# YichengDWu/tinyedm

Hardware: AMD Instinct MI355X
Metric: train imgs/sec CIFAR-10 32x32 bf16 (higher is better)
Workload: dtype bf16; 1 GPU; CIFAR-10 32x32 unconditional EDM2 U-Net (conf/cifar10.yaml, 35.6M params) full training step: diffuse+embed+denoiser fwd/bwd+loss+grad all-reduce+Adam+EMA; per_gpu_batch=128, global_batch=128, parallelism=dp1, conditional=False, step_launch=hipGraph replay, collective=none

## Files before the change

include/tinyedm_hip.h:

```cpp
#ifndef TINYEDM_HIP_H
#define TINYEDM_HIP_H
#ifdef __cplusplus
extern "C" {
#endif

typedef struct ihipStream_t* edm_stream_t;

int edm_version(void);
const char* edm_last_error(void);
int edm_init(int device);
int edm_graph_replay_safe(void);
typedef struct {
  unsigned step, seed_lo, seed_hi, reserved;
  float lr, ema_beta, grad_scale, bc1, bc2sqrt, pad[3];
} edm_step_params;

int edm_conv_igemm(const void* X, const void* Wp, void* Y, const void* R, float alpha, float beta, int B, int H,
                   int W, int Cin, int Cout, int taps, edm_stream_t stream);
int edm_conv_igemm_v2(const void* X, const void* Wp, void* Y, const void* R, float alpha, float beta, int B, int H,
                      int W, int Cin, int Cout, int taps, edm_stream_t stream);
int edm_conv_igemm_v6(const void* X, const void* Wp, void* Y, const void* R, float alpha, float beta, int B, int H,
                      int W, int Cin, int Cout, int taps, edm_stream_t stream);
int edm_conv_igemm_s(const void* X, const void* Wp, void* Y, const void* R, float alpha, float beta, int B, int H,
                     int W, int Cin, int Cout, int taps, edm_stream_t stream);
// ... 68 lines not shown
} edm_finish_item;
long edm_wgrad_finish_multi_table_bytes(void);
int edm_wgrad_finish_multi(const edm_finish_item* items, int n, void* table_host, void* table_dev, int defer_upload,
                           edm_stream_t stream);

int edm_attention_fwd(const void* qkv, void* y, int B, int N, int C, int heads, edm_stream_t stream);
int edm_attention_bwd(const void* qkv, const void* y, const void* gy, void* gqkv, int B, int N, int C, int heads,
                      edm_stream_t stream);

int edm_attention_qkv_supported(int N, int C, int heads);
int edm_attention_qkv_fwd(const void* x, const void* Wqkv, void* y, void* stat, int B, int N, int C, int heads,
                          int heads_per_wg, edm_stream_t stream);
int edm_attention_qkv_bwd(const void* x, const void* y, const void* gout, const void* stat, const void* Wqkv,
                          const void* Wd_out, void* gqkv, float alpha, int B, int N, int C, int heads, int heads_per_wg,
                          edm_stream_t stream);

int edm_pixelnorm_silu_fwd(const void* x, void* xn, void* a, float* dsave, long P, int C, edm_stream_t stream);
int edm_pixelnorm_silu_bwd(const void* xn, const float* dsave, const void* gxn, float gxn_scale, const void* ga,
                           const void* gadd, void* gx, long P, int C, edm_stream_t stream);
int edm_pool_pixelnorm_silu_fwd(const void* x, void* xn, void* a, float* dsave, int B, int Hp, int Wp, int C,
                                edm_stream_t stream);
int edm_pool_pixelnorm_silu_bwd(const void* xn, const float* dsave, const void* gxn, float gxn_scale, const void* ga,
                                const void* gadd, void* gx, int B, int Hp, int Wp, int C, edm_stream_t stream);
int edm_silu_fwd(const void* x, void* a, long n, edm_stream_t stream);
int edm_silu_bwd(const void* x, const void* ga, const void* gextra, float extra_scale, void* gx, long n,
                 edm_stream_t stream);
int edm_axpby(const void* a, float alpha, const void* b, float beta, void* out, long n, edm_stream_t stream);
int edm_mod_silu_drop_fwd(const void* r, const float* lin, long lin_stride, const float* gain, void* a, int B, int HW,
                          int C, float pdrop, unsigned long long seed, unsigned sub, unsigned step, const void* dyn,
                          edm_stream_t stream);
int edm_mod_silu_drop_bwd(const void* r, const float* lin, long lin_stride, const float* gain, const void* ga, void* gr,
                          float* gm, float* glin, long glin_stride, float* ggain, int B, int HW, int C, float pdrop,
                          unsigned long long seed, unsigned sub, unsigned step, const void* dyn, edm_stream_t stream);
int edm_mod_silu_drop_bwd_raw(const void* r, const float* lin, long lin_stride, const float* gain, const void* ga, void* gr,
                              float* gm, long gm_stride, int B, int HW, int C, float pdrop, unsigned long long seed,
                              unsigned sub, unsigned step, const void* dyn, edm_stream_t stream);
int edm_dropout_mask(unsigned char* mask, long n, float pdrop, unsigned long long seed, unsigned sub, unsigned step,
                     edm_stream_t stream);
int edm_pool2(const void* x, void* y, int B, int Hout, int Wout, int C, float scale, edm_stream_t stream);
int edm_up2(const void* x, const void* add, void* y, int B, int Hout, int Wout, int C, float scale, edm_stream_t stream);
int edm_up2_silu(const void* x, void* y, void* a, int B, int Hout, int Wout, int C, edm_stream_t stream);
int edm_reduce_hw(const void* x, long x_stride, const void* y, long y_stride, float* out, int B, int HW, int C,
                  float scale, edm_stream_t stream);
int edm_scalelong_fwd(const float* mean, const float* W1h, const float* W2h, float* gate, float* z1save, int B, int C,
                      int R, edm_stream_t stream);
int edm_scalelong_bwd(const float* mean, const float* W1h, const float* W2h, const float* gate, const float* z1save,
// ... 200 lines not shown
```

tinyedm_amd/_lib.py:

```python
import ctypes
import os

_HERE = os.path.dirname(os.path.abspath(__file__))
LIB_PATH = os.environ.get("EDM_LIB_PATH") or os.path.join(_HERE, "libtinyedm_hip.so")

P, I, L, F = ctypes.c_void_p, ctypes.c_int, ctypes.c_long, ctypes.c_float
U, U64 = ctypes.c_uint, ctypes.c_ulonglong

SIGNATURES = {
    "edm_version": [],
    "edm_last_error": [],
    "edm_init": [I],
    "edm_graph_replay_safe": [],
    "edm_pixelnorm_silu_fwd": [P, P, P, P, L, I, P],
    "edm_pixelnorm_silu_bwd": [P, P, P, F, P, P, P, L, I, P],
    "edm_pool_pixelnorm_silu_fwd": [P, P, P, P, I, I, I, I, P],
    "edm_pool_pixelnorm_silu_bwd": [P, P, P, F, P, P, P, I, I, I, I, P],
    "edm_up2_silu": [P, P, P, I, I, I, I, P],
    "edm_silu_fwd": [P, P, L, P],
    "edm_silu_bwd": [P, P, P, F, P, L, P],
    "edm_axpby": [P, F, P, F, P, L, P],
    "edm_mod_silu_drop_fwd": [P, P, L, P, P, I, I, I, F, U64, U, U, P, P],
    "edm_mod_silu_drop_bwd": [P, P, L, P, P, P, P, P, L, P, I, I, I, F, U64, U, U, P, P],
    "edm_mod_silu_drop_bwd_raw": [P, P, L, P, P, P, P, L, I, I, I, F, U64, U, U, P, P],
    "edm_dropout_mask": [P, L, F, U64, U, U, P],
    "edm_pool2": [P, P, I, I, I, I, F, P],
    "edm_up2": [P, P, P, I, I, I, I, F, P],
    "edm_reduce_hw": [P, L, P, L, P, I, I, I, F, P],
    "edm_scalelong_fwd": [P, P, P, P, P, I, I, I, P],
    "edm_scalelong_bwd": [P, P, P, P, P, P, P, P, P, I, I, I, P],
    "edm_skip_gate_fwd": [P, P, P, P, P, P, I, I, I, I, P],
    "edm_skip_gate_bwd": [P, L, I, P, P, P, P, P, P, P, P, P, P, I, I, I, I, P],
    "edm_skip_gate_wgrad_multi": [P, I, P, P, I, P],
    "edm_skip_gate_wgrad_multi_table_bytes": [],
    "edm_skip_gate_fwd_multi": [P, I, P, P, I, P],
    "edm_skip_gate_fwd_multi_table_bytes": [],
    "edm_skip_gate_bwd_multi": [P, I, P, P, I, P],
    "edm_skip_half_bwd_multi": [P, I, P, P, I, P],
    "edm_skip_gate_bwd_multi_table_bytes": [],
    "edm_concat_gate_fwd": [P, P, P, P, P, I, I, I, I, P],
# ... 193 lines not shown
```

tinyedm_amd/csrc/elementwise.hip:

```cpp
#include "common.h"
#include <stdarg.h>
#include <stdio.h>

static thread_local char g_err[512] = "";
extern "C" void edm_set_error(const char* fmt, ...) {
  va_list ap;
  va_start(ap, fmt);
  vsnprintf(g_err, sizeof(g_err), fmt, ap);
  va_end(ap);
}
extern "C" const char* edm_last_error() { return g_err; }
extern "C" int edm_version() { return 1; }

static inline int cdiv(long a, long b) { return (int)((a + b - 1) / b); }
static inline int grid_for(long work, int block, int cap = 256 * 16) {
  long g = (work + block - 1) / block;
  if (g > cap) g = cap;
  if (g < 1) g = 1;
  return (int)g;
}

template <int LPP, bool POOL = false>
__global__ __launch_bounds__(256) void k_pnorm_silu_fwd(const bf16* __restrict__ x, bf16* __restrict__ xn,
                                                          bf16* __restrict__ a, float* __restrict__ dsave, int P,
// ... 35 lines not shown
      }
    }
    ss = group_sum<LPP>(ss);
    const float d = NORM_EPS + sqrtf(ss) * rsC;
    const float inv = 1.0f / d;
#pragma unroll
    for (int it = 0; it < 2; ++it) {
      const int c8 = lig + it * LPP;
      if (pv && c8 < CL) {
        float o[8], s[8];
#pragma unroll
        for (int i = 0; i < 8; ++i) {
          o[i] = (float)(bf16)(v[it][i] * inv);
          s[i] = mp_silu_b(o[i]);
        }
        store8(xn + p * C + c8 * 8, o);
        store8(a + p * C + c8 * 8, s);
      }
    }
    if (pv && lig == 0) dsave[p] = d;
  }
}

template <int LPP, bool UP = false>
__global__ __launch_bounds__(256) void k_pnorm_silu_bwd(const bf16* __restrict__ xn, const float* __restrict__ dsave,
                                                          const bf16* __restrict__ gxn, float gs,
                                                          const bf16* __restrict__ ga, const bf16* __restrict__ gadd,
                                                          bf16* __restrict__ gx, int P, int C, int Hp = 0, int Wp = 0) {
  constexpr int GPW = 64 / LPP;
  const int lane = threadIdx.x & 63, wave = threadIdx.x >> 6;
  const int lig = lane % LPP, grp = lane / LPP;
  const int CL = C >> 3;
  const long stride = (long)gridDim.x * 4 * GPW;
  for (long p0 = ((long)blockIdx.x * 4 + wave) * GPW; p0 < P; p0 += stride) {
    const long p = p0 + grp;
    const bool pv = p < P;
    float y[2][8], g[2][8];
    float dot = 0.f;
#pragma unroll
    for (int it = 0; it < 2; ++it) {
      const int c8 = lig + it * LPP;
      if (pv && c8 < CL) {
        load8(xn + p * C + c8 * 8, y[it]);
        float t[8];
        if (gxn) {
          load8(gxn + p * C + c8 * 8, t);
#pragma unroll
          for (int i = 0; i < 8; ++i) g[it][i] = gs * t[i];
        } else {
#pragma unroll
          for (int i = 0; i < 8; ++i) g[it][i] = 0.f;
// ... 8 lines not shown
      }
    }
    dot = group_sum<LPP>(dot);
    float d = pv ? dsave[p] : 1.f;
    float s = d - NORM_EPS;
    float coef = s > 0.f ? dot * d / ((float)C * s) : 0.f;
    float inv = 1.0f / d;
#pragma unroll
    for (int it = 0; it < 2; ++it) {
      const int c8 = lig + it * LPP;
      if (pv && c8 < CL) {
        float o[8];
#pragma unroll
        for (int i = 0; i < 8; ++i) o[i] = (g[it][i] - y[it][i] * coef) * inv;
        if constexpr (UP) {
          const int w = (int)(p % Wp);
          const long t2 = p / Wp;
          const int h = (int)(t2 % Hp);
          const long b = t2 / Hp;
          const long e0 = ((b * 2 * Hp + 2 * h) * 2 * Wp + 2 * w) * C + c8 * 8;
          const long row = (long)2 * Wp * C;
#pragma unroll
          for (int i = 0; i < 8; ++i) o[i] = 0.25f * (float)(bf16)o[i];
#pragma unroll
          for (int q = 0; q < 4; ++q) {
            const long e = e0 + (q >> 1) * row + (q & 1) * C;
            float r[8];
#pragma unroll
            for (int i = 0; i < 8; ++i) r[i] = o[i];
            if (gadd) {
              float t[8];
              load8(gadd + e, t);
#pragma unroll
              for (int i = 0; i < 8; ++i) r[i] += t[i];
            }
            store8(gx + e, r);
          }
          continue;
        }
        if (gadd) {
          float t[8];
          load8(gadd + p * C + c8 * 8, t);
#pragma unroll
          for (int i = 0; i < 8; ++i) o[i] += t[i];
        }
        store8(gx + p * C + c8 * 8, o);
      }
    }
  }
}

static int pick_lpp(int C) {
  int cl = C / 8;
  return cl <= 16 ? 16 : (cl <= 32 ? 32 : 64);
}

extern "C" int edm_pixelnorm_silu_fwd(const void* x, void* xn, void* a, float* dsave, long P, int C,
                                      hipStream_t st) {
  EDM_REQUIRE(P > 0 && P < (1L << 31) && C > 0 && C % 8 == 0 && C <= 1024, "pixelnorm_silu_fwd: bad P=%ld C=%d", P, C);
  int lpp = pick_lpp(C);
  int gpw = 64 / lpp;
  int grid = grid_for(P, 4 * gpw);
#define L(N) hipLaunchKernelGGL(k_pnorm_silu_fwd<N>, dim3(grid), dim3(256), 0, st, (const bf16*)x, (bf16*)xn, (bf16*)a, dsave, (int)P, C)
// ... 23 lines not shown
  EDM_REQUIRE(xn && dsave && gx && B > 0 && Hp > 0 && Wp > 0 && C > 0 && C % 8 == 0 && C <= 1024 &&
                  (long)B * Hp * Wp < (1L << 31), "pool_pixelnorm_silu_bwd: bad args");
  const long P = (long)B * Hp * Wp;
  int lpp = pick_lpp(C);
  int gpw = 64 / lpp;
  int grid = grid_for(P, 4 * gpw);
#define L(N) hipLaunchKernelGGL((k_pnorm_silu_bwd<N, true>), dim3(grid), dim3(256), 0, st, (const bf16*)xn, dsave, (const bf16*)gxn, gxn_scale, (const bf16*)ga, (const bf16*)gadd, (bf16*)gx, (int)P, C, Hp, Wp)
  if (lpp == 16) L(16); else if (lpp == 32) L(32); else L(64);
#undef L
  EDM_CHECK_LAUNCH("pool_pixelnorm_silu_bwd");
  return EDM_OK;
}

extern "C" int edm_pixelnorm_silu_bwd(const void* xn, const float* dsave, const void* gxn, float gxn_scale,
                                      const void* ga, const void* gadd, void* gx, long P, int C, hipStream_t st) {
  EDM_REQUIRE(P > 0 && P < (1L << 31) && C > 0 && C % 8 == 0 && C <= 1024, "pixelnorm_silu_bwd: bad P=%ld C=%d", P, C);
  int lpp = pick_lpp(C);
  int gpw = 64 / lpp;
  int grid = grid_for(P, 4 * gpw);
#define L(N) hipLaunchKernelGGL(k_pnorm_silu_bwd<N>, dim3(grid), dim3(256), 0, st, (const bf16*)xn, dsave, (const bf16*)gxn, gxn_scale, (const bf16*)ga, (const bf16*)gadd, (bf16*)gx, (int)P, C)
  if (lpp == 16) L(16); else if (lpp == 32) L(32); else L(64);
#undef L
  EDM_CHECK_LAUNCH("pixelnorm_silu_bwd");
  return EDM_OK;
}

__global__ void k_silu_fwd(const bf16* __restrict__ x, bf16* __restrict__ a, long n8) {
  for (long i = (long)blockIdx.x * blockDim.x + threadIdx.x; i < n8; i += (long)gridDim.x * blockDim.x) {
    float v[8];
    load8(x + i * 8, v);
#pragma unroll
    for (int j = 0; j < 8; ++j) v[j] = mp_silu_b(v[j]);
    store8(a + i * 8, v);
  }
}
__global__ void k_silu_bwd(const bf16* __restrict__ x, const bf16* __restrict__ ga, const bf16* __restrict__ ge,
                           float s, bf16* __restrict__ gx, long n8) {
  for (long i = (long)blockIdx.x * blockDim.x + threadIdx.x; i < n8; i += (long)gridDim.x * blockDim.x) {
    float v[8], g[8], e[8];
    load8(x + i * 8, v);
    load8(ga + i * 8, g);
    if (ge) load8(ge + i * 8, e);
#pragma unroll
    for (int j = 0; j < 8; ++j) g[j] = mp_silu_grad_b(v[j]) * g[j] + (ge ? s * e[j] : 0.f);
    store8(gx + i * 8, g);
  }
// ... 649 lines not shown
  int k = 0;
  const int n = g->n;
  while (k + 1 < n && (int)blockIdx.x >= g->it[k + 1].blk0) ++k;
  const SgbItem it = g->it[k];
  const int C = g->C, b = (int)blockIdx.x - it.blk0;
  skip_gate_bwd_body(it.gcat, it.gs, it.skip, it.W1, it.W2, it.gate, it.z1, it.gmean, it.ws, it.HW, C, it.R, b);
  if (it.gskip == nullptr) return;
  __syncthreads();
  const int CLs = C >> 3;
  const float inv_hw = 1.0f / (float)it.HW;
  const bf16* __restrict__ gc = it.gcat + (long)b * it.HW * it.gs;
  bf16* __restrict__ out = it.gskip + (long)b * it.HW * C;
  const float* gp0 = it.gate + (long)b * C;
  const float* mp0 = it.gmean + (long)b * C;
  const int n8 = it.HW * CLs;
  for (int i = threadIdx.x; i < n8; i += blockDim.x) {
    const int cs = (i % CLs) * 8;
    const int pix = i / CLs;
    float v[8];
    load8(gc + (long)pix * it.gs + cs, v);
    const float* gp = gp0 + cs;
    const float* mp = mp0 + cs;
#pragma unroll
    for (int j = 0; j < 8; ++j) v[j] = v[j] * gp[j] + mp[j] * inv_hw;
    store8(out + (long)pix * C + cs, v);
  }
}
__device__ __forceinline__ void skip_gate_wgrad_body(const float* __restrict__ ws, const float* __restrict__ mean,
                                                     float* __restrict__ gW1, float* __restrict__ gW2, int B, int C, int R,
                                                     int CT, int BC, int blk) {
  extern __shared__ __attribute__((aligned(16))) float sm[];
  float* A = sm;
  float* Bm = sm + 4 * BC;
  const int W = C + 2 * R;
  const bool second = blk >= CT;
  const int c0 = (second ? blk - CT : blk) * 4;
  const int ncol = second ? C + 1 : C;
  const int boff = second ? C : C + R;
  constexpr int MAXO = 16;
  float acc[MAXO];
#pragma unroll
  for (int k = 0; k < MAXO; ++k) acc[k] = 0.f;
  for (int b0 = 0; b0 < B; b0 += BC) {
    const int nb = min(BC, B - b0);
    if (b0) __syncthreads();
    for (int i = threadIdx.x; i < 4 * nb; i += blockDim.x) {
      const int b = b0 + (i >> 2), c = c0 + (i & 3);
// ... 277 lines not shown
    const float* gp = gate + (long)b * Cs + cs;
#pragma unroll
    for (int j = 0; j < 8; ++j) v[j] = (float)(bf16)(v[j] * gp[j]);
    store8(cat + pix * ld + Ci + cs, v);
    if (sil) {
#pragma unroll
      for (int j = 0; j < 8; ++j) v[j] = mp_silu_b(v[j]);
      store8(sil + pix * ld + Ci + cs, v);
    }
  }
}
__device__ __forceinline__ void skip_half_bwd_body(const bf16* __restrict__ gcs, const float* __restrict__ gate,
                                                   const float* __restrict__ gmean, bf16* __restrict__ gskip, int HW, int Cs,
                                                   long n8, float inv_hw, long first, long stride) {
  const int CLs = Cs >> 3;
  for (long i = first; i < n8; i += stride) {
    const int cs = (int)(i % CLs) * 8;
    const int b = (int)((i / CLs) / HW);
    float v[8];
    load8(gcs + i * 8, v);
    const float* gp = gate + (long)b * Cs + cs;
    const float* mp = gmean + (long)b * Cs + cs;
#pragma unroll
    for (int j = 0; j < 8; ++j) v[j] = v[j] * gp[j] + mp[j] * inv_hw;
    store8(gskip + i * 8, v);
  }
}
__global__ void k_skip_half_bwd(const bf16* __restrict__ gcs, const float* __restrict__ gate,
                                const float* __restrict__ gmean, bf16* __restrict__ gskip, int HW, int Cs, long n8,
                                float inv_hw) {
  skip_half_bwd_body(gcs, gate, gmean, gskip, HW, Cs, n8, inv_hw, (long)blockIdx.x * blockDim.x + threadIdx.x,
                     (long)gridDim.x * blockDim.x);
}
struct ShbItem {
  const bf16* gcs;
  const float* gate;
  const float* gmean;
  bf16* gskip;
  long n8;
  float inv_hw;
  int HW, Cs, blk0, nblk, pad;
};
struct ShbGroup {
  ShbItem it[MAXSGF];
  int n, pad[3];
};
__global__ void k_skip_half_bwd_multi(const ShbGroup* __restrict__ g) {
// ... 338 lines not shown
```

tinyedm_amd/networks.py:

```python
from __future__ import annotations

import math
import os
from typing import Optional

import numpy as np
import torch
import torch.nn as nn
from torch import Tensor

from . import ops

bf16, f32 = torch.bfloat16, torch.float32


class _Rng:
    seed: int = 42
    step: int = 0
    dyn = None


rng = _Rng()


# ... 75 lines not shown
            if len(pend) >= FIN_GROUP:
                _flush_fin(key)
            _queue_backward_end(w.device)
            return None
        g = ops.wgrad_finish(slabs, w.data, self._taps(), I, perm=self._perm, scale=scale)
        return g.view_as(w)


WGRAD_STREAM = os.environ.get("EDM_WGRAD_STREAM", "1") != "0"
W3_GROUP = max(0, min(ops.W3_MAX_LAYERS, int(os.environ.get("EDM_W3_GROUP", "16"))))
W3_TAIL = max(0, int(os.environ.get("EDM_W3_TAIL", "0")))
_w3_seen = {}
_w3_total = {}
W3_MAXPIX = int(os.environ.get("EDM_W3_MAXPIX", str(1 << 18)))
FIN_GROUP = 40
W1_GROUP = max(0, min(16, int(os.environ.get("EDM_W1_GROUP", "16"))))
_w1_pending = {}
_bwd_end_queued = set()
MOD_DEFER_UNFUSED = os.environ.get("EDM_MOD_DEFER_UNFUSED", "1") != "0"
SG_MULTI = os.environ.get("EDM_SG_MULTI", "1") != "0"
SG_HALVES = os.environ.get("EDM_SG_HALVES", "1") != "0"
SG_BWD_MULTI = os.environ.get("EDM_SG_BWD_MULTI", "1") != "0"
SG_DEFER = os.environ.get("EDM_SG_DEFER", "1") != "0"
_sg_pending = {}
_w3_pending = {}
_fin_pending = {}


def _run_on_side(device, fn, tensors=()):
    if WGRAD_STREAM:
        side = ops.side_stream(device)
        side.wait_stream(torch.cuda.current_stream())
        with torch.cuda.stream(side):
            fn()
        for t in tensors:
            t.record_stream(side)
    else:
        fn()


def _flush_w3(key):
    items = _w3_pending.pop(key, None)
    if not items:
        return
    dev = items[0][0].weight.device
    args = [(x, dy, m.weight.data, m.weight.grad, m._perm, scale, True) for m, x, dy, scale in items]
# ... 632 lines not shown
        mod = ctx.mod
        gout = gout.contiguous()
        a, b = _mp_coeffs(0.5)
        if ctx.fused:
            x, stat, y, wd_qkv, wd_out, wf_qkv = ctx.saved_tensors
            if stat is None:
                raise RuntimeError("tinyedm_amd: attention backward without the forward's softmax statistics (the forward ran "
                                   "under torch.no_grad())")
            gqkv = ops.attention_qkv_bwd(x, y, gout, stat, wf_qkv, wd_out, mod.num_heads, alpha=b)
        else:
            x, qkv, y, wd_qkv, wd_out = ctx.saved_tensors
            gy = ops.conv_igemm(gout, wd_out, 1, alpha=b)
            gqkv = ops.attention_bwd(qkv, y, gy, mod.num_heads)
        gw_out = _wgrad(mod.out_conv, y, gout, 1, b)
        gx = ops.conv_igemm(gqkv, wd_qkv, 1, residual=gout, alpha=1.0, beta=a)
        gw_qkv = _wgrad(mod.qkv_conv, x, gqkv, 1)
        return gx, gw_qkv, gw_out, None, None, None


class _ResBlockFn(torch.autograd.Function):

    @staticmethod
    def forward(ctx, u, emb, w1x1, w1, w2, wemb, gain, blk, lin_view, glin_view, token, s_pre=None, alias=False,
                gm_view=None, skip=None, w_sl1=None, w_sl2=None, pre=None, dest=None, pool=False, gate_pre=None):
        enc = blk.is_encoder
        ctx.set_materialize_grads(False)
        has1 = w1x1 is not None
        taps = 9
        wf1, wd1, _ = blk.conv_3x3_1.packs()
        wf2, wd2, _ = blk.conv_3x3_2.packs()
        batched = lin_view is not None
        weh = None if batched else blk.embed.packs()[2]
        wd11 = None
        ctx.has_skip = skip is not None
        if skip is not None:
            sl = blk.cat_factor
            ctx.sgb = None
            if gate_pre is not None:
                mean, gate, z1, w1h, w2h, ctx.sgb, halves = gate_pre
            else:
                w1h, w2h = sl.layer1.packs()[2], sl.layer2.packs()[2]
                mean, gate, z1 = ops.skip_gate_fwd(skip, w1h, w2h)
            ctx.Ci = u.shape[-1]
            if pre is not None and pre[0].shape[-1] == u.shape[-1] + skip.shape[-1] and pre[0].data_ptr() == u.data_ptr():
                cat, s_pre = pre
                if not (gate_pre is not None and halves == cat.data_ptr()):
                    ops.skip_half_fwd(skip, gate, cat, s_pre)
            else:
                cat, s_pre = ops.concat_gate_fwd(u.contiguous(), skip, gate, True)
            u = cat
# ... 75 lines not shown
            deferred = MOD_DEFER_UNFUSED and ctx.gm_view is not None and gdirect
            ga2 = ops.conv_igemm(gout, wd2, 9, alpha=b)
            gr1, glin, ggain = ops.mod_silu_drop_bwd(r1, lin, gain, ga2, pdrop, seed, sub, step, glin_out=glin_out,
                                                        ggain_out=ggain_out, dyn=dyn, gm_out=ctx.gm_view if deferred else None)
            if deferred:
                gp._edm_deferred = True
        if gdirect:
            ggain = None
            if not deferred:
                for hook in getattr(gp, "_edm_hooks", ()):
                    hook(gp)
        gw2 = _wgrad(blk.conv_3x3_2, a2, gout, 9, b)
        gwemb = gemb = gtoken = None
        if ctx.batched:
            gtoken = ops.zeros_f32((1,), gout.device) if ctx.has_token else None
        else:
            dweh = ops.linear_wgrad(glin, emb)
            gwemb = blk.embed.finish_grad(dweh.view(1, 1, *dweh.shape))
            gemb = ops.linear_dgrad(glin, weh) if ctx.needs_input_grad[1] else None
        fuse = ops.FUSE_MOD and ops.IGEMM_VERSION == 0 and not enc
        gs = None if fuse else ops.conv_igemm(gr1, wd1, 9)
        gw1 = _wgrad(blk.conv_3x3_1, s, gr1, 9)
        gw11 = None
        if enc and ctx.pool:
            gu = ops.pool_pixelnorm_silu_bwd(xn, dsave, gout, a, gs, gadd=g_alias)
            g_alias = None
        elif enc:
            gx = ops.pixelnorm_silu_bwd(xn, dsave, gout, a, gs, gadd=None if has1 else g_alias)
            if has1:
                gw11 = _wgrad(blk.conv_1x1, u, gx, 1)
                gu = ops.conv_igemm(gx, wd11, 1, residual=g_alias, alpha=1.0, beta=1.0 if g_alias is not None else 0.0)
            else:
                gu = gx
            g_alias = None
        else:
            if has1:
                t = ops.conv3x3_silubwd(gr1, wd1, u) if fuse else ops.silu_bwd(u, gs)
                if ctx.has_skip:
                    Ci = ctx.Ci
                    B_, H_, W_, Ct = u.shape
                    gu = torch.empty(B_, H_, W_, Ci, device=u.device, dtype=bf16)
                    gcs = torch.empty(B_, H_, W_, Ct - Ci, device=u.device, dtype=bf16)
                    ops.conv_igemm(gout, wd11, 1, residual=t, alpha=a, beta=1.0, split=(Ci, gu, gcs))
                else:
                    gu = ops.conv_igemm(gout, wd11, 1, residual=t, alpha=a, beta=1.0)
                    gcs = None
                gw11 = _wgrad(blk.conv_1x1, u, gout, 1, a)
            else:
                gu = ops.conv3x3_silubwd(gr1, wd1, u, gout, a) if fuse else ops.silu_bwd(u, gs, gout, a)
                gcs = None
        gskip = gwsl1 = gwsl2 = None
        if ctx.has_skip:
            skip, mean, gate, z1, w1h, w2h = ctx.skip_saved
            Ci = ctx.Ci
            sl = blk.cat_factor
            wsl = (sl.layer1.weight, sl.layer2.weight)
            defer = SG_DEFER and all(w.grad is not None and getattr(w, "_edm_direct", False) for w in wsl)
            sgb = getattr(ctx, "sgb", None)
            queued = False
            if gcs is None:
                gmean, *gws = ops.skip_gate_bwd(gu, Ci, skip, mean, w1h, w2h, gate, z1, defer_wgrad=defer)
                gu, gskip = ops.concat_gate_bwd(gu, gate, gmean, Ci)
            elif defer and sgb is not None and SG_BWD_MULTI:
                gskip = torch.empty_like(gcs)
                sgb.pending.append((gcs, skip, w1h, w2h, gate, z1, gskip, sl, mean))
                queued = True
            else:
                gmean, *gws = ops.skip_gate_bwd(gcs, 0, skip, mean, w1h, w2h, gate, z1, defer_wgrad=defer)
                gskip = ops.skip_half_bwd(gcs, gate, gmean)
            if defer:
                if not queued:
                    _sg_pending.setdefault(wsl[0].device.index, []).append((sl, gws[0], mean, w1h.shape[0]))
                wsl[0]._edm_deferred = wsl[1]._edm_deferred = True
                _queue_backward_end(wsl[0].device)
            else:
                gw1h, gw2h = gws
                gwsl1 = sl.layer1.finish_grad(gw1h.view(1, 1, *gw1h.shape))
                gwsl2 = sl.layer2.finish_grad(gw2h.view(1, 1, *gw2h.shape))
            if sgb is not None:
                sgb.arrived += 1
                if sgb.arrived == sgb.expected:
                    sgb.flush()
        if g_alias is not None:
            gu = ops.axpby(gu, 1.0, g_alias, 1.0)
        return (gu, gemb, gw11, gw1, gw2, gwemb, ggain, None, None, None, gtoken, None, None, None, gskip, gwsl1, gwsl2,
                None, None, None, None)


_rng_sub_counter = [0]


class _BlockBase(nn.Module):
    is_encoder = True

    def _common(self, out_channels, embedding_dim, attention, num_heads, dropout_rate):
        self.conv_3x3_2 = Conv2d(out_channels, out_channels, 3)
        self.dropout = nn.Dropout(dropout_rate)
        self.attention = CosineAttention(out_channels, num_heads) if attention else nn.Identity()
        self.embed = Linear(embedding_dim, out_channels)
        self.embed.weight._edm_late = True
        self.gain = nn.Parameter(torch.ones(()))
        _rng_sub_counter[0] += 1
        self.rng_sub = _rng_sub_counter[0]

    def _res(self, u: Tensor, embedding: Tensor, lin=None, s_pre=None, alias=False, skip=None, dest=None, pool=False,
             gate=None):
        w11 = self.conv_1x1.weight if isinstance(self.conv_1x1, Conv2d) else None
        has_attn = isinstance(self.attention, CosineAttention)
        sk = ()
        if skip is not None or dest is not None or pool:
            cf = self.cat_factor if skip is not None else None
            sk = (skip, cf.layer1.weight if cf is not None else None, cf.layer2.weight if cf is not None else None,
                  getattr(u, "_edm_cat", None) if skip is not None else None, None if has_attn else dest, bool(pool),
                  gate if skip is not None else None)
        if lin is None:
            out = _ResBlockFn.apply(u, embedding, w11, self.conv_3x3_1.weight, self.conv_3x3_2.weight,
                                    self.embed.weight, self.gain, self, None, None, None, s_pre, alias, None, *sk)
        else:
            lin_view, glin_view, token, gm_view = lin
            out = _ResBlockFn.apply(u, None, w11, self.conv_3x3_1.weight, self.conv_3x3_2.weight, None, self.gain,
                                    self, lin_view, glin_view, token, s_pre, alias, gm_view, *sk)
        ualias = None
        if alias:
            out, ualias = out
        if has_attn:
            out = self.attention.forward_nhwc(out, dest)
        elif dest is not None and out.data_ptr() == dest[0].data_ptr():
            out._edm_cat = dest
        return (out, ualias) if alias else out


_SPLIT_EVAL = [False]
F32_FUSE_OUT = os.environ.get("EDM_F32_FUSE_OUT", "1") != "0"


def _split_ok(mod) -> bool:
    return bool(_SPLIT_EVAL[0]) and isinstance(mod, _WNBase) and mod.weight.shape[1] % 32 == 0 and mod.weight.shape[0] % 8 == 0
# ... 54 lines not shown
    if x.dtype == bf16 and getattr(x, "_edm_nhwc", False):
        return x, False
    return ops.nchw_to_nhwc_bf16(x.float().contiguous()), True


def _tag(x: Tensor) -> Tensor:
    x._edm_nhwc = True
    return x


class EncoderBlock(_BlockBase):
    is_encoder = True

    def __init__(self, in_channels: int, out_channels: int, embedding_dim: int, down: bool, attention: bool,
                 num_heads: int = 4, dropout_rate: float = 0.0, add_factor: float = 0.3):
        super().__init__()
        self.dropout_rate = dropout_rate
        self.add_factor = add_factor
        self.resample = DownSample() if down else nn.Identity()
        self.conv_1x1 = Conv2d(in_channels, out_channels, 1) if in_channels != out_channels else nn.Identity()
        self.conv_3x3_1 = Conv2d(out_channels, out_channels, 3)
        self._common(out_channels, embedding_dim, attention, num_heads, dropout_rate)

    def forward(self, input: Tensor, embedding: Tensor, _lin=None, _alias: bool = False, _dest=None):
        x, conv = _as_nhwc(input)
        ualias = None
        emb = None if _lin is not None else _emb32(embedding, x.shape[0])
        if (isinstance(self.resample, DownSample) and FUSE_RESAMPLE and not isinstance(self.conv_1x1, Conv2d)
                and x.shape[-1] <= 1024 and x.shape[1] % 2 == 0 and x.shape[2] % 2 == 0):
            out = self._res(x, emb, _lin, alias=_alias, pool=True, dest=_dest)
            if _alias:
                out, ualias = out
        else:
            if isinstance(self.resample, DownSample):
                if _alias:
                    x, ualias = _ResampleFn.apply(x, False, True)
                else:
                    x = _ResampleFn.apply(x, False)
            if _alias and ualias is None:
                out, ualias = self._res(x, emb, _lin, alias=True, dest=_dest)
            else:
                out = self._res(x, emb, _lin, dest=_dest)
        if conv:
            out = ops.nhwc_bf16_to_nchw(out).to(input.dtype)
        else:
            cat_pre = getattr(out, "_edm_cat", None)
            out = _tag(out)
            if cat_pre is not None:
                out._edm_cat = cat_pre
        return (out, _tag(ualias)) if _alias else out

    def forward_f32(self, x: Tensor, lin: Tensor, want=None):
        pairs = _split_ok(self.conv_3x3_1)
        if (F32_FUSE_OUT and isinstance(self.resample, DownSample) and not isinstance(self.conv_1x1, Conv2d)
                and x.shape[-1] <= 1024):
            xn, s = ops.f32_pool_pixelnorm_silu(x, pairs=pairs)
        else:
            if isinstance(self.resample, DownSample):
                x = ops.f32_pool2(x)
            if isinstance(self.conv_1x1, Conv2d):
                x = _conv_f32(self.conv_1x1, x, 1)
            xn, s = ops.f32_pixelnorm_silu(x, pairs=pairs)
        return _res_f32(self, xn, s, lin, want)


class DecoderBlock(_BlockBase):
    is_encoder = False

    def __init__(self, in_channels: int, out_channels: int, embedding_dim: int, up: bool, attention: bool,
                 num_heads: int = 4, skip_channels: int = 0, dropout_rate: float = 0.0, add_factor: float = 0.3):
        super().__init__()
        self.add_factor = add_factor
        self.dropout_rate = dropout_rate
        self.cat_factor = ScaleLong(skip_channels) if skip_channels > 0 else None
        self.resample = UpSample() if up else nn.Identity()
        total = in_channels + skip_channels
        self.conv_1x1 = Conv2d(total, out_channels, 1) if total != out_channels else nn.Identity()
        self.conv_3x3_1 = Conv2d(total, out_channels, 3)
        self._common(out_channels, embedding_dim, attention, num_heads, dropout_rate)

    def _gate_in_block(self) -> bool:
        return (FUSE_CAT and SKIP_GATE_FUSED and not isinstance(self.resample, UpSample)
                and isinstance(self.conv_1x1, Conv2d) and self.cat_factor is not None)

    def forward(self, input: Tensor, embedding: Tensor, skip: Tensor | None = None, _lin=None, _dest=None, _gate=None) -> Tensor:
        x, conv = _as_nhwc(input)
        s_pre = None
        if skip is not None and FUSE_CAT and SKIP_GATE_FUSED and not isinstance(self.resample, UpSample) \
                and isinstance(self.conv_1x1, Conv2d):
            assert self.cat_factor is not None
            sk, _ = _as_nhwc(skip)
            out = self._res(x, None if _lin is not None else _emb32(embedding, x.shape[0]), _lin, skip=sk, dest=_dest,
                            gate=_gate)
            return ops.nhwc_bf16_to_nchw(out).to(input.dtype) if conv else _tag(out)
        if skip is not None:
            assert self.cat_factor is not None
            sk, _ = _as_nhwc(skip)
            fuse_silu = not isinstance(self.resample, UpSample)
            x = _ConcatGateFn.apply(x, sk, self.cat_factor.layer1.weight, self.cat_factor.layer2.weight, self.cat_factor,
                                    fuse_silu)
            if fuse_silu:
                x, s_pre = x
        if skip is None and not isinstance(self.resample, UpSample):
            pre = getattr(x, "_edm_cat", None)
            if pre is not None and pre[0].data_ptr() == x.data_ptr() and pre[0].shape == x.shape:
                s_pre = pre[1]
        if isinstance(self.resample, UpSample):
            if FUSE_RESAMPLE:
                x, s_pre = _ResampleFn.apply(x, True, False, True)
            else:
                x = _ResampleFn.apply(x, True)
                s_pre = None
        out = self._res(x, None if _lin is not None else _emb32(embedding, x.shape[0]), _lin, s_pre, dest=_dest)
        return ops.nhwc_bf16_to_nchw(out).to(input.dtype) if conv else _tag(out)

    @staticmethod
# ... 420 lines not shown
            return D.to(noisy_image.dtype)
        reset_backward_state()
        if torch.is_grad_enabled():
            global FORWARD_EPOCH
            FORWARD_EPOCH += 1
        with torch.no_grad():
            self._prep_all((noisy_image.shape[0], noisy_image.shape[2], noisy_image.shape[3]))
        noisy = noisy_image.float().contiguous()
        B = noisy.shape[0]
        sig = sigma.detach().float().flatten().contiguous()
        emb = _emb32(embedding, B)

        blocks = self._res_blocks()
        lin_all, glin_all, token, gm_all = _EmbedAllFn.apply(emb, self, *[b.embed.weight for b in blocks])
        lins, off = {}, 0
        for k, b in enumerate(blocks):
            C = b.embed.weight.shape[0]
            lins[b] = (lin_all[:, off:off + C], glin_all[:, off:off + C], token if k == 0 else None,
                       None if gm_all is None else gm_all[:, off:off + C])
            off += C

        x = _ConvInFn.apply(noisy, sig, self.conv_in.weight, self)
        skips = []
        dec = list(zip(self.decoder_blocks, self.skip_connections))
        enc = list(self.encoder_blocks)
        for k, block in enumerate(enc):
            dest = None
            if k + 1 == len(enc) and dec and not dec[0][1]:
                dest = self._silu_dest(block, dec[0][0], x, 1, down=isinstance(block.resample, DownSample))
            x, x_in = block(_tag(x), None, _lin=lins[block], _alias=True, _dest=dest)
            skips.append(x_in)
        skips.append(x)
        dests = _decoder_dests_impl(dec, skips, x) if FUSE_CAT and SKIP_GATE_FUSED else {}
        gates = self._decoder_gates(dec, skips, dests) if SG_MULTI else {}
        for i, (block, has_skip) in enumerate(dec):
            skip = skips.pop() if has_skip else None
            dest = dests.get(i)
            if dest is not None:
                pass
            elif i + 1 < len(dec):
                dest = self._silu_dest(block, dec[i + 1][0], x, 2 if isinstance(block.resample, UpSample) else 1)
            xin = _tag(x)
            cat_pre = getattr(x, "_edm_cat", None)
            if cat_pre is not None:
                xin._edm_cat = cat_pre
            x = block(xin, None, _tag(skip) if has_skip else None, _lin=lins[block], _dest=dest, _gate=gates.get(block))
        D = _ConvOutFn.apply(x, self.conv_out.weight, self.gain_out, noisy, sig, self)
        if self.training:
            rng.step += 1
        return D.to(noisy_image.dtype)


class _SgbPass:

    def __init__(self, expected: int):
        self.expected, self.arrived, self.pending = expected, 0, []

    def flush(self):
        items, self.pending = self.pending, []
        self.arrived = 0
        if not items:
            return
        by_c = {}
        for it in items:
            by_c.setdefault(it[1].shape[-1], []).append(it)
        halves = []
        for group in by_c.values():
            for k0 in range(0, len(group), 32):
                part = group[k0:k0 + 32]
                res = ops.skip_gate_bwd_multi([(gcs, 0, skip, w1h, w2h, gate, z1) + ((gskip,) if SG_HALVES else ())
                                               for gcs, skip, w1h, w2h, gate, z1, gskip, _, _ in part])
                for (gcs, skip, w1h, w2h, gate, z1, gskip, sl, mean), (gmean, ws) in zip(part, res):
                    if not SG_HALVES:
                        halves.append((gcs, gate, gmean, gskip))
                    _sg_pending.setdefault(sl.layer1.weight.device.index, []).append((sl, ws, mean, w1h.shape[0]))
        for k0 in range(0, len(halves), 32):
            ops.skip_half_bwd_multi(halves[k0:k0 + 32])


def _decoder_dests_impl(dec, skips, x):
    out = {}
    st = list(skips)
    h, w = x.shape[1], x.shape[2]
    for i, (block, has_skip) in enumerate(dec):
        if has_skip:
            st.pop()
        if isinstance(block.resample, UpSample):
            h, w = 2 * h, 2 * w
        if i + 1 < len(dec) and dec[i + 1][1]:
            nxt = dec[i + 1][0]
            if not isinstance(nxt.resample, UpSample) and isinstance(nxt.conv_1x1, Conv2d):
                Ct = block.conv_3x3_2.weight.shape[0] + st[-1].shape[-1]
                out[i] = (torch.empty(x.shape[0], h, w, Ct, device=x.device, dtype=bf16),
                          torch.empty(x.shape[0], h, w, Ct, device=x.device, dtype=bf16))
    return out


# ... 46 lines not shown
```

tinyedm_amd/ops.py:

```python
import contextlib
import ctypes
import functools
import math
import os
import types
from typing import Optional

import torch

from . import _lib

bf16, f32 = torch.bfloat16, torch.float32

PROFILE = None


class _prof:
    def __init__(self, name, flops, nbytes):
        self.name, self.flops, self.nbytes = name, flops, nbytes

    def __enter__(self):
        if PROFILE is not None:
            self.s = torch.cuda.Event(enable_timing=True)
            self.e = torch.cuda.Event(enable_timing=True)
# ... 306 lines not shown
def pool_pixelnorm_silu_fwd(x):
    B, H, W, C = _nhwc(x, "x")
    if H % 2 or W % 2 or C > 1024:
        raise ValueError("pool_pixelnorm_silu_fwd: H, W even and C <= 1024 required")
    xn = torch.empty(B, H // 2, W // 2, C, device=x.device, dtype=bf16)
    a = torch.empty_like(xn)
    d = torch.empty(B * (H // 2) * (W // 2), device=x.device, dtype=f32)
    _lib.call("edm_pool_pixelnorm_silu_fwd", _p(x), _p(xn), _p(a), _p(d), B, H // 2, W // 2, C, _stream())
    return xn, a, d


def pool_pixelnorm_silu_bwd(xn, d, gxn, gxn_scale, ga, gadd=None):
    B, H, W, C = _nhwc(xn, "xn")
    _chk(d, f32, "d", (B * H * W,))
    if gxn is not None:
        _chk(gxn, bf16, "gxn", xn.shape)
    if ga is not None:
        _chk(ga, bf16, "ga", xn.shape)
    if gadd is not None:
        _chk(gadd, bf16, "gadd", (B, 2 * H, 2 * W, C))
    gx = torch.empty(B, 2 * H, 2 * W, C, device=xn.device, dtype=bf16)
    _lib.call("edm_pool_pixelnorm_silu_bwd", _p(xn), _p(d), _p(gxn), float(gxn_scale), _p(ga), _p(gadd), _p(gx), B, H, W, C,
              _stream())
    return gx


def up2_silu(x):
    B, H, W, C = _nhwc(x, "x")
    y = torch.empty(B, 2 * H, 2 * W, C, device=x.device, dtype=bf16)
    a = torch.empty_like(y)
    _lib.call("edm_up2_silu", _p(x), _p(y), _p(a), B, 2 * H, 2 * W, C, _stream())
    return y, a


def silu_fwd(x):
    _chk(x, bf16, "x")
    a = torch.empty_like(x)
    _lib.call("edm_silu_fwd", _p(x), _p(a), x.numel(), _stream())
    return a


def silu_bwd(x, ga, gextra=None, extra_scale=1.0):
    _chk(x, bf16, "x")
    _chk(ga, bf16, "ga", x.shape)
    if gextra is not None:
        _chk(gextra, bf16, "gextra", x.shape)
# ... 1797 lines not shown
```

Measured before the change: 10230 img/s.

## Defer skip-gradient formation into encoder pixelnorm-SiLU backward kernels

Instead of materializing the U-Net skip gradient (gcs*gate + gmean/HW) in a separate pass and then re-reading it in the encoder block's pixelnorm/SiLU backward, the decoder now leaves gcs, gate and gmean on a token. The encoder's backward computes the skip gradient inline through new lazy variants of the pixelnorm-SiLU backward kernels, with and without pooling. This removes one bf16 write and read of the skip gradient tensor per skip connection, plus a kernel launch. It adds token bookkeeping, falls back to the old path when hooks or a 1x1 conv are present, and raises an error if the gradient arrives as an unexpected tensor.

```diff
diff --git a/include/tinyedm_hip.h b/include/tinyedm_hip.h
--- a/include/tinyedm_hip.h
+++ b/include/tinyedm_hip.h
@@ -114,6 +114,12 @@
                                 edm_stream_t stream);
 int edm_pool_pixelnorm_silu_bwd(const void* xn, const float* dsave, const void* gxn, float gxn_scale, const void* ga,
                                 const void* gadd, void* gx, int B, int Hp, int Wp, int C, edm_stream_t stream);
+int edm_pixelnorm_silu_bwd_lazy(const void* xn, const float* dsave, const void* gxn, float gxn_scale, const void* ga,
+                                const void* gcs, long gcs_ld, const float* gate, const float* gmean, void* gx, int B, int HW,
+                                int C, edm_stream_t stream);
+int edm_pool_pixelnorm_silu_bwd_lazy(const void* xn, const float* dsave, const void* gxn, float gxn_scale, const void* ga,
+                                     const void* gcs, long gcs_ld, const float* gate, const float* gmean, void* gx, int B,
+                                     int Hp, int Wp, int C, edm_stream_t stream);
 int edm_silu_fwd(const void* x, void* a, long n, edm_stream_t stream);
 int edm_silu_bwd(const void* x, const void* ga, const void* gextra, float extra_scale, void* gx, long n,
                  edm_stream_t stream);
diff --git a/tinyedm_amd/_lib.py b/tinyedm_amd/_lib.py
--- a/tinyedm_amd/_lib.py
+++ b/tinyedm_amd/_lib.py
@@ -16,6 +16,8 @@
     "edm_pixelnorm_silu_bwd": [P, P, P, F, P, P, P, L, I, P],
     "edm_pool_pixelnorm_silu_fwd": [P, P, P, P, I, I, I, I, P],
     "edm_pool_pixelnorm_silu_bwd": [P, P, P, F, P, P, P, I, I, I, I, P],
+    "edm_pixelnorm_silu_bwd_lazy": [P, P, P, F, P, P, L, P, P, P, I, I, I, P],
+    "edm_pool_pixelnorm_silu_bwd_lazy": [P, P, P, F, P, P, L, P, P, P, I, I, I, I, P],
     "edm_up2_silu": [P, P, P, I, I, I, I, P],
     "edm_silu_fwd": [P, P, L, P],
     "edm_silu_bwd": [P, P, P, F, P, L, P],
diff --git a/tinyedm_amd/csrc/elementwise.hip b/tinyedm_amd/csrc/elementwise.hip
--- a/tinyedm_amd/csrc/elementwise.hip
+++ b/tinyedm_amd/csrc/elementwise.hip
@@ -81,11 +81,31 @@
   }
 }
 
-template <int LPP, bool UP = false>
+struct LazySkip {
+  const bf16* gcs;
+  long ld;
+  const float* gate;
+  const float* gmean;
+  float inv_hw;
+  int HW;
+};
+__device__ __forceinline__ float skip_grad(float gcs, float gate, float gmean, float inv_hw) {
+  return __fmaf_rn(gcs, gate, gmean * inv_hw);
+}
+__device__ __forceinline__ void load8f(const float* p, float (&f)[8]) {
+  const f32x4 a = *reinterpret_cast<const f32x4*>(p), b = *reinterpret_cast<const f32x4*>(p + 4);
+#pragma unroll
+  for (int i = 0; i < 4; ++i) {
+    f[i] = a[i];
+    f[4 + i] = b[i];
+  }
+}
+template <int LPP, bool UP = false, bool LAZY = false>
 __global__ __launch_bounds__(256) void k_pnorm_silu_bwd(const bf16* __restrict__ xn, const float* __restrict__ dsave,
                                                           const bf16* __restrict__ gxn, float gs,
                                                           const bf16* __restrict__ ga, const bf16* __restrict__ gadd,
-                                                          bf16* __restrict__ gx, int P, int C, int Hp = 0, int Wp = 0) {
+                                                          bf16* __restrict__ gx, int P, int C, int Hp = 0, int Wp = 0,
+                                                          LazySkip lz = LazySkip{}) {
   constexpr int GPW = 64 / LPP;
   const int lane = threadIdx.x & 63, wave = threadIdx.x >> 6;
   const int lig = lane % LPP, grp = lane / LPP;
@@ -140,13 +160,26 @@
           const long row = (long)2 * Wp * C;
 #pragma unroll
           for (int i = 0; i < 8; ++i) o[i] = 0.25f * (float)(bf16)o[i];
+          float lg[8], lm[8];
+          if constexpr (LAZY) {
+            load8f(lz.gate + b * C + c8 * 8, lg);
+            load8f(lz.gmean + b * C + c8 * 8, lm);
+#pragma unroll
+            for (int i = 0; i < 8; ++i) asm volatile("" : "+v"(o[i]));
+          }
 #pragma unroll
           for (int q = 0; q < 4; ++q) {
             const long e = e0 + (q >> 1) * row + (q & 1) * C;
             float r[8];
 #pragma unroll
             for (int i = 0; i < 8; ++i) r[i] = o[i];
-            if (gadd) {
+            if constexpr (LAZY) {
+              const long pe = (b * 2 * Hp + 2 * h + (q >> 1)) * 2 * Wp + 2 * w + (q & 1);
+              float t[8];
+              load8(lz.gcs + pe * lz.ld + c8 * 8, t);
+#pragma unroll
+              for (int i = 0; i < 8; ++i) r[i] += (float)(bf16)skip_grad(t[i], lg[i], lm[i], lz.inv_hw);
+            } else if (gadd) {
               float t[8];
               load8(gadd + e, t);
 #pragma unroll
@@ -156,7 +189,18 @@
           }
           continue;
         }
-        if (gadd) {
+        if constexpr (LAZY) {
+          const long b = (int)p / lz.HW;
+          float t[8], lg[8], lm[8];
+          load8(lz.gcs + p * lz.ld + c8 * 8, t);
+          load8f(lz.gate + b * C + c8 * 8, lg);
+          load8f(lz.gmean + b * C + c8 * 8, lm);
+#pragma unroll
+          for (int i = 0; i < 8; ++i) {
+            asm volatile("" : "+v"(o[i]));
+            o[i] += (float)(bf16)skip_grad(t[i], lg[i], lm[i], lz.inv_hw);
+          }
+        } else if (gadd) {
           float t[8];
           load8(gadd + p * C + c8 * 8, t);
 #pragma unroll
@@ -226,6 +270,47 @@
   if (lpp == 16) L(16); else if (lpp == 32) L(32); else L(64);
 #undef L
   EDM_CHECK_LAUNCH("pixelnorm_silu_bwd");
+  return EDM_OK;
+}
+
+static bool lazy_args_ok(const void* gcs, long gcs_ld, const float* gate, const float* gmean, int C) {
+  return gcs && gate && gmean && gcs_ld >= C && gcs_ld % 8 == 0 && ((uintptr_t)gcs & 15) == 0 && ((uintptr_t)gate & 15) == 0 &&
+         ((uintptr_t)gmean & 15) == 0;
+}
+extern "C" int edm_pixelnorm_silu_bwd_lazy(const void* xn, const float* dsave, const void* gxn, float gxn_scale,
+                                           const void* ga, const void* gcs, long gcs_ld, const float* gate,
+                                           const float* gmean, void* gx, int B, int HW, int C, hipStream_t st) {
+  EDM_REQUIRE(xn && dsave && gx && B > 0 && HW > 0 && (long)B * HW < (1L << 31) && C > 0 && C % 8 == 0 && C <= 1024,
+              "pixelnorm_silu_bwd_lazy: bad B=%d HW=%d C=%d", B, HW, C);
+  EDM_REQUIRE(lazy_args_ok(gcs, gcs_ld, gate, gmean, C), "pixelnorm_silu_bwd_lazy: bad gcs / gate / gmean (ld %ld)", gcs_ld);
+  const long P = (long)B * HW;
+  const LazySkip lz{(const bf16*)gcs, gcs_ld, gate, gmean, 1.0f / (float)HW, HW};
+  int lpp = pick_lpp(C);
+  int gpw = 64 / lpp;
+  int grid = grid_for(P, 4 * gpw);
+#define L(N) hipLaunchKernelGGL((k_pnorm_silu_bwd<N, false, true>), dim3(grid), dim3(256), 0, st, (const bf16*)xn, dsave, (const bf16*)gxn, gxn_scale, (const bf16*)ga, (const bf16*)nullptr, (bf16*)gx, (int)P, C, 0, 0, lz)
+  if (lpp == 16) L(16); else if (lpp == 32) L(32); else L(64);
+#undef L
+  EDM_CHECK_LAUNCH("pixelnorm_silu_bwd_lazy");
+  return EDM_OK;
+}
+extern "C" int edm_pool_pixelnorm_silu_bwd_lazy(const void* xn, const float* dsave, const void* gxn, float gxn_scale,
+                                                const void* ga, const void* gcs, long gcs_ld, const float* gate,
+                                                const float* gmean, void* gx, int B, int Hp, int Wp, int C,
+                                                hipStream_t st) {
+  EDM_REQUIRE(xn && dsave && gx && B > 0 && Hp > 0 && Wp > 0 && C > 0 && C % 8 == 0 && C <= 1024 &&
+                  (long)B * Hp * Wp * 4 < (1L << 31), "pool_pixelnorm_silu_bwd_lazy: bad args");
+  EDM_REQUIRE(lazy_args_ok(gcs, gcs_ld, gate, gmean, C), "pool_pixelnorm_silu_bwd_lazy: bad gcs / gate / gmean (ld %ld)", gcs_ld);
+  const long P = (long)B * Hp * Wp;
+  const int HW = 4 * Hp * Wp;
+  const LazySkip lz{(const bf16*)gcs, gcs_ld, gate, gmean, 1.0f / (float)HW, HW};
+  int lpp = pick_lpp(C);
+  int gpw = 64 / lpp;
+  int grid = grid_for(P, 4 * gpw);
+#define L(N) hipLaunchKernelGGL((k_pnorm_silu_bwd<N, true, true>), dim3(grid), dim3(256), 0, st, (const bf16*)xn, dsave, (const bf16*)gxn, gxn_scale, (const bf16*)ga, (const bf16*)nullptr, (bf16*)gx, (int)P, C, Hp, Wp, lz)
+  if (lpp == 16) L(16); else if (lpp == 32) L(32); else L(64);
+#undef L
+  EDM_CHECK_LAUNCH("pool_pixelnorm_silu_bwd_lazy");
   return EDM_OK;
 }
 
@@ -921,7 +1006,7 @@
     const float* gp = gp0 + cs;
     const float* mp = mp0 + cs;
 #pragma unroll
-    for (int j = 0; j < 8; ++j) v[j] = v[j] * gp[j] + mp[j] * inv_hw;
+    for (int j = 0; j < 8; ++j) v[j] = skip_grad(v[j], gp[j], mp[j], inv_hw);
     store8(out + (long)pix * C + cs, v);
   }
 }
@@ -1245,7 +1330,7 @@
     const float* gp = gate + (long)b * Cs + cs;
     const float* mp = gmean + (long)b * Cs + cs;
 #pragma unroll
-    for (int j = 0; j < 8; ++j) v[j] = v[j] * gp[j] + mp[j] * inv_hw;
+    for (int j = 0; j < 8; ++j) v[j] = skip_grad(v[j], gp[j], mp[j], inv_hw);
     store8(gskip + i * 8, v);
   }
 }
diff --git a/tinyedm_amd/networks.py b/tinyedm_amd/networks.py
--- a/tinyedm_amd/networks.py
+++ b/tinyedm_amd/networks.py
@@ -121,6 +121,7 @@
 SG_HALVES = os.environ.get("EDM_SG_HALVES", "1") != "0"
 SG_BWD_MULTI = os.environ.get("EDM_SG_BWD_MULTI", "1") != "0"
 SG_DEFER = os.environ.get("EDM_SG_DEFER", "1") != "0"
+SG_LAZY = os.environ.get("EDM_SG_LAZY", "1") != "0"
 _sg_pending = {}
 _w3_pending = {}
 _fin_pending = {}
@@ -799,10 +800,14 @@
 
     @staticmethod
     def forward(ctx, u, emb, w1x1, w1, w2, wemb, gain, blk, lin_view, glin_view, token, s_pre=None, alias=False,
-                gm_view=None, skip=None, w_sl1=None, w_sl2=None, pre=None, dest=None, pool=False, gate_pre=None):
+                gm_view=None, skip=None, w_sl1=None, w_sl2=None, pre=None, dest=None, pool=False, gate_pre=None,
+                skip_tok=None):
         enc = blk.is_encoder
         ctx.set_materialize_grads(False)
         has1 = w1x1 is not None
+        ctx.skip_tok = skip_tok
+        if skip_tok is not None and enc:
+            skip_tok.lazy_ok = bool(alias) and not has1
         taps = 9
         wf1, wd1, _ = blk.conv_3x3_1.packs()
         wf2, wd2, _ = blk.conv_3x3_2.packs()
@@ -924,7 +929,12 @@
         gs = None if fuse else ops.conv_igemm(gr1, wd1, 9)
         gw1 = _wgrad(blk.conv_3x3_1, s, gr1, 9)
         gw11 = None
-        if enc and ctx.pool:
+        lazy = _take_skip_grad(ctx.skip_tok, g_alias, can_lazy=not has1) if enc else None
+        if lazy is not None:
+            bwd = ops.pool_pixelnorm_silu_bwd_lazy if ctx.pool else ops.pixelnorm_silu_bwd_lazy
+            gu = bwd(xn, dsave, gout, a, gs, *lazy)
+            g_alias = None
+        elif enc and ctx.pool:
             gu = ops.pool_pixelnorm_silu_bwd(xn, dsave, gout, a, gs, gadd=g_alias)
             g_alias = None
         elif enc:
@@ -965,7 +975,7 @@
                 gu, gskip = ops.concat_gate_bwd(gu, gate, gmean, Ci)
             elif defer and sgb is not None and SG_BWD_MULTI:
                 gskip = torch.empty_like(gcs)
-                sgb.pending.append((gcs, skip, w1h, w2h, gate, z1, gskip, sl, mean))
+                sgb.queue((gcs, skip, w1h, w2h, gate, z1, gskip, sl, mean), ctx.skip_tok)
                 queued = True
             else:
                 gmean, *gws = ops.skip_gate_bwd(gcs, 0, skip, mean, w1h, w2h, gate, z1, defer_wgrad=defer)
@@ -986,7 +996,7 @@
         if g_alias is not None:
             gu = ops.axpby(gu, 1.0, g_alias, 1.0)
         return (gu, gemb, gw11, gw1, gw2, gwemb, ggain, None, None, None, gtoken, None, None, None, gskip, gwsl1, gwsl2,
-                None, None, None, None)
+                None, None, None, None, None)
 
 
 _rng_sub_counter = [0]
@@ -1006,15 +1016,15 @@
         self.rng_sub = _rng_sub_counter[0]
 
     def _res(self, u: Tensor, embedding: Tensor, lin=None, s_pre=None, alias=False, skip=None, dest=None, pool=False,
-             gate=None):
+             gate=None, skip_tok=None):
         w11 = self.conv_1x1.weight if isinstance(self.conv_1x1, Conv2d) else None
         has_attn = isinstance(self.attention, CosineAttention)
         sk = ()
-        if skip is not None or dest is not None or pool:
+        if skip is not None or dest is not None or pool or skip_tok is not None:
             cf = self.cat_factor if skip is not None else None
             sk = (skip, cf.layer1.weight if cf is not None else None, cf.layer2.weight if cf is not None else None,
                   getattr(u, "_edm_cat", None) if skip is not None else None, None if has_attn else dest, bool(pool),
-                  gate if skip is not None else None)
+                  gate if skip is not None else None, skip_tok)
         if lin is None:
             out = _ResBlockFn.apply(u, embedding, w11, self.conv_3x3_1.weight, self.conv_3x3_2.weight,
                                     self.embed.weight, self.gain, self, None, None, None, s_pre, alias, None, *sk)
@@ -1115,13 +1125,13 @@
         self.conv_3x3_1 = Conv2d(out_channels, out_channels, 3)
         self._common(out_channels, embedding_dim, attention, num_heads, dropout_rate)
 
-    def forward(self, input: Tensor, embedding: Tensor, _lin=None, _alias: bool = False, _dest=None):
+    def forward(self, input: Tensor, embedding: Tensor, _lin=None, _alias: bool = False, _dest=None, _skip_tok=None):
         x, conv = _as_nhwc(input)
         ualias = None
         emb = None if _lin is not None else _emb32(embedding, x.shape[0])
         if (isinstance(self.resample, DownSample) and FUSE_RESAMPLE and not isinstance(self.conv_1x1, Conv2d)
                 and x.shape[-1] <= 1024 and x.shape[1] % 2 == 0 and x.shape[2] % 2 == 0):
-            out = self._res(x, emb, _lin, alias=_alias, pool=True, dest=_dest)
+            out = self._res(x, emb, _lin, alias=_alias, pool=True, dest=_dest, skip_tok=_skip_tok if _alias else None)
             if _alias:
                 out, ualias = out
         else:
@@ -1131,7 +1141,7 @@
                 else:
                     x = _ResampleFn.apply(x, False)
             if _alias and ualias is None:
-                out, ualias = self._res(x, emb, _lin, alias=True, dest=_dest)
+                out, ualias = self._res(x, emb, _lin, alias=True, dest=_dest, skip_tok=_skip_tok)
             else:
                 out = self._res(x, emb, _lin, dest=_dest)
         if conv:
@@ -1176,7 +1186,8 @@
         return (FUSE_CAT and SKIP_GATE_FUSED and not isinstance(self.resample, UpSample)
                 and isinstance(self.conv_1x1, Conv2d) and self.cat_factor is not None)
 
-    def forward(self, input: Tensor, embedding: Tensor, skip: Tensor | None = None, _lin=None, _dest=None, _gate=None) -> Tensor:
+    def forward(self, input: Tensor, embedding: Tensor, skip: Tensor | None = None, _lin=None, _dest=None, _gate=None,
+                _skip_tok=None) -> Tensor:
         x, conv = _as_nhwc(input)
         s_pre = None
         if skip is not None and FUSE_CAT and SKIP_GATE_FUSED and not isinstance(self.resample, UpSample) \
@@ -1184,7 +1195,7 @@
             assert self.cat_factor is not None
             sk, _ = _as_nhwc(skip)
             out = self._res(x, None if _lin is not None else _emb32(embedding, x.shape[0]), _lin, skip=sk, dest=_dest,
-                            gate=_gate)
+                            gate=_gate, skip_tok=_skip_tok)
             return ops.nhwc_bf16_to_nchw(out).to(input.dtype) if conv else _tag(out)
         if skip is not None:
             assert self.cat_factor is not None
@@ -1651,19 +1662,24 @@
 
         x = _ConvInFn.apply(noisy, sig, self.conv_in.weight, self)
         skips = []
+        toks = []
+        want_tok = SG_LAZY and torch.is_grad_enabled()
         dec = list(zip(self.decoder_blocks, self.skip_connections))
         enc = list(self.encoder_blocks)
         for k, block in enumerate(enc):
             dest = None
             if k + 1 == len(enc) and dec and not dec[0][1]:
                 dest = self._silu_dest(block, dec[0][0], x, 1, down=isinstance(block.resample, DownSample))
-            x, x_in = block(_tag(x), None, _lin=lins[block], _alias=True, _dest=dest)
+            toks.append(_SkipGrad() if want_tok else None)
+            x, x_in = block(_tag(x), None, _lin=lins[block], _alias=True, _dest=dest, _skip_tok=toks[-1])
             skips.append(x_in)
         skips.append(x)
+        toks.append(None)
         dests = _decoder_dests_impl(dec, skips, x) if FUSE_CAT and SKIP_GATE_FUSED else {}
         gates = self._decoder_gates(dec, skips, dests) if SG_MULTI else {}
         for i, (block, has_skip) in enumerate(dec):
             skip = skips.pop() if has_skip else None
+            tok = toks.pop() if has_skip else None
             dest = dests.get(i)
             if dest is not None:
                 pass
@@ -1673,17 +1689,68 @@
             cat_pre = getattr(x, "_edm_cat", None)
             if cat_pre is not None:
                 xin._edm_cat = cat_pre
-            x = block(xin, None, _tag(skip) if has_skip else None, _lin=lins[block], _dest=dest, _gate=gates.get(block))
+            x = block(xin, None, _tag(skip) if has_skip else None, _lin=lins[block], _dest=dest, _gate=gates.get(block),
+                      _skip_tok=tok)
         D = _ConvOutFn.apply(x, self.conv_out.weight, self.gain_out, noisy, sig, self)
         if self.training:
             rng.step += 1
         return D.to(noisy_image.dtype)
 
 
+class _SkipGrad:
+    QUEUED, LAZY, FILLED = 1, 2, 3
+    __slots__ = ("lazy_ok", "state", "ph", "gcs", "gate", "gmean", "sgb")
+
+    def __init__(self):
+        self.lazy_ok = False
+        self.clear()
+
+    def clear(self):
+        self.state = self.ph = self.gcs = self.gate = self.gmean = self.sgb = None
+
+
+def _take_skip_grad(tok, g_alias, can_lazy):
+    if tok is None or tok.state is None:
+        return None
+    mine = g_alias is not None and g_alias.data_ptr() == tok.ph.data_ptr() and g_alias.shape == tok.ph.shape
+    if mine and tok.state == _SkipGrad.QUEUED:
+        tok.sgb.flush()
+    state, ph, lazy = tok.state, tok.ph, (tok.gcs, tok.gate, tok.gmean)
+    if state != _SkipGrad.LAZY:
+        if mine:
+            tok.clear()
+        return None
+    tok.clear()
+    if not mine:
+        raise RuntimeError("tinyedm_amd: the gradient of a U-Net skip reached its encoder block as another tensor than the one "
+                           "the decoder block handed out, whose values were left to this block to form (a second consumer of "
+                           "the skip, or a hook that replaced the gradient before the decoder's backward ran): set EDM_SG_LAZY=0")
+    if not can_lazy:
+        ops.skip_half_bwd_multi([(*lazy, ph)])
+        return None
+    return lazy
+
+
+def _skip_observed(skip) -> bool:
+    return bool(getattr(skip, "_backward_hooks", None)) or bool(getattr(skip, "retains_grad", False))
+
+
 class _SgbPass:
 
     def __init__(self, expected: int):
         self.expected, self.arrived, self.pending = expected, 0, []
+
+    def queue(self, item, tok):
+        sl = item[7]
+        if any(it[7] is sl for it, _ in self.pending):
+            for _, t in self.pending:
+                if t is not None:
+                    t.clear()
+            self.pending, self.arrived = [], 0
+        if tok is not None:
+            tok.clear()
+            tok.state, tok.ph, tok.sgb = _SkipGrad.QUEUED, item[6], self
+        self.pending.append((item, tok))
 
     def flush(self):
         items, self.pending = self.pending, []
@@ -1692,16 +1759,22 @@
             return
         by_c = {}
         for it in items:
-            by_c.setdefault(it[1].shape[-1], []).append(it)
+            by_c.setdefault(it[0][1].shape[-1], []).append(it)
         halves = []
         for group in by_c.values():
             for k0 in range(0, len(group), 32):
                 part = group[k0:k0 + 32]
-                res = ops.skip_gate_bwd_multi([(gcs, 0, skip, w1h, w2h, gate, z1) + ((gskip,) if SG_HALVES else ())
-                                               for gcs, skip, w1h, w2h, gate, z1, gskip, _, _ in part])
-                for (gcs, skip, w1h, w2h, gate, z1, gskip, sl, mean), (gmean, ws) in zip(part, res):
-                    if not SG_HALVES:
-                        halves.append((gcs, gate, gmean, gskip))
+                lazy = [SG_LAZY and tok is not None and tok.lazy_ok and not _skip_observed(it[1]) for it, tok in part]
+                res = ops.skip_gate_bwd_multi([(gcs, 0, skip, w1h, w2h, gate, z1) + ((gskip,) if SG_HALVES and not lz else ())
+                                               for ((gcs, skip, w1h, w2h, gate, z1, gskip, _, _), _), lz in zip(part, lazy)])
+                for ((gcs, skip, w1h, w2h, gate, z1, gskip, sl, mean), tok), lz, (gmean, ws) in zip(part, lazy, res):
+                    if lz:
+                        tok.state, tok.gcs, tok.gate, tok.gmean = _SkipGrad.LAZY, gcs, gate, gmean
+                    else:
+                        if tok is not None:
+                            tok.state = _SkipGrad.FILLED
+                        if not SG_HALVES:
+                            halves.append((gcs, gate, gmean, gskip))
                     _sg_pending.setdefault(sl.layer1.weight.device.index, []).append((sl, ws, mean, w1h.shape[0]))
         for k0 in range(0, len(halves), 32):
             ops.skip_half_bwd_multi(halves[k0:k0 + 32])
diff --git a/tinyedm_amd/ops.py b/tinyedm_amd/ops.py
--- a/tinyedm_amd/ops.py
+++ b/tinyedm_amd/ops.py
@@ -352,6 +352,46 @@
     gx = torch.empty(B, 2 * H, 2 * W, C, device=xn.device, dtype=bf16)
     _lib.call("edm_pool_pixelnorm_silu_bwd", _p(xn), _p(d), _p(gxn), float(gxn_scale), _p(ga), _p(gadd), _p(gx), B, H, W, C,
               _stream())
+    return gx
+
+
+def _lazy_skip_args(gcs, gate, gmean, shape):
+    B, H, W, C = shape
+    if not isinstance(gcs, torch.Tensor) or not gcs.is_cuda or gcs.dtype != bf16 or tuple(gcs.shape) != (B, H, W, C):
+        raise ValueError(f"gcs: expected a bf16 GPU tensor of shape {(B, H, W, C)}")
+    ld = gcs.stride(2)
+    if gcs.stride(3) != 1 or ld < C or ld % 8 or gcs.stride(1) != W * ld or gcs.stride(0) != H * W * ld or gcs.data_ptr() % 16:
+        raise ValueError("gcs: pixel rows of one stride (a multiple of 8 elements, >= C), 16-byte aligned")
+    _chk(gate, f32, "gate", (B, C))
+    _chk(gmean, f32, "gmean", (B, C))
+    return ld
+
+
+def pixelnorm_silu_bwd_lazy(xn, d, gxn, gxn_scale, ga, gcs, gate, gmean):
+    B, H, W, C = _nhwc(xn, "xn")
+    _chk(d, f32, "d", (B * H * W,))
+    if gxn is not None:
+        _chk(gxn, bf16, "gxn", xn.shape)
+    if ga is not None:
+        _chk(ga, bf16, "ga", xn.shape)
+    ld = _lazy_skip_args(gcs, gate, gmean, (B, H, W, C))
+    gx = torch.empty_like(xn)
+    _lib.call("edm_pixelnorm_silu_bwd_lazy", _p(xn), _p(d), _p(gxn), float(gxn_scale), _p(ga), _p(gcs), ld, _p(gate),
+              _p(gmean), _p(gx), B, H * W, C, _stream())
+    return gx
+
+
+def pool_pixelnorm_silu_bwd_lazy(xn, d, gxn, gxn_scale, ga, gcs, gate, gmean):
+    B, H, W, C = _nhwc(xn, "xn")
+    _chk(d, f32, "d", (B * H * W,))
+    if gxn is not None:
+        _chk(gxn, bf16, "gxn", xn.shape)
+    if ga is not None:
+        _chk(ga, bf16, "ga", xn.shape)
+    ld = _lazy_skip_args(gcs, gate, gmean, (B, 2 * H, 2 * W, C))
+    gx = torch.empty(B, 2 * H, 2 * W, C, device=xn.device, dtype=bf16)
+    _lib.call("edm_pool_pixelnorm_silu_bwd_lazy", _p(xn), _p(d), _p(gxn), float(gxn_scale), _p(ga), _p(gcs), ld, _p(gate),
+              _p(gmean), _p(gx), B, H, W, C, _stream())
     return gx
 
 
```

Result: no change. 10300 img/s (median of 6 runs) (+0.7%).
